# FintanH/rust-crdt

Hardware: AMD Instinct MI355X
Metric: replica-merges/sec (whole node) + achieved HBM GB/s as % of MI355X peak (higher is better)
Workload: dtype u64

## Files before the change

rust-crdt_amd/csrc/common.hpp:

```cpp
#pragma once

#include <hip/hip_runtime.h>

#include <cstdint>
#include <cstdio>
#include <algorithm>
#include <cstring>
#include <map>
#include <string>
#include <vector>

#include "crdt_gpu.h"
#include "shard_host.hpp"

namespace crdt {

using u64 = unsigned long long;
using u64x2 = unsigned long long __attribute__((ext_vector_type(2)));

constexpr int kWave = 64;

#ifndef CRDT_APPLY_WPE
#define CRDT_APPLY_WPE 0
#endif
#if CRDT_APPLY_WPE
#define CRDT_APPLY_ATTR __attribute__((amdgpu_waves_per_eu(CRDT_APPLY_WPE)))
#else
#define CRDT_APPLY_ATTR
#endif
constexpr int kBlock = 256;

struct KernelTimer {
  double total_ms = 0.0;
  uint64_t launches = 0;
};

struct Tune {
  int lub_blocks_per_cu = 1;
  int lub_grid = 0;
  int lub_persist_grid = 0;
  int lub_chunk_bytes = 512 << 10;
  int lub_min_steps = 16;
  int lub_interleave = 0;
  int lub_unroll = 8;
  int lub_nt = 1;
  int orswot_blocks_per_cu = 2;
  int orswot_unroll = 1;
  int orswot_mpt = 4;
  int merge_blocks_per_cu = 2;
  int merge_rows = 1;
  int map_glds = 1;
  int map_chunk = 16;
  int map_ring = 2;
  int map_spec = 1;
  int map_nt = 0;
  int map_scan2 = 0;
  int map_scan3 = 1;
  int map_rs = 1;
  int map_batch = 1;
  int map_sh = 0;
  int map_lazyv = 1;
  int map_st = 0;
  int shagree = 0;
  int map_diag = 0;
  int rows_blocks_per_cu = 0;
  int apply_hot_slots = 8;
  int map_apply_hot = 1 << 20;
  int map_forget_vec2 = 1;
  int map_pair_reg = 1;
  int pair_rows = 256;
  int pair_ur = 8;
  int pair_occ = 1;
  int map_forget_bpc = 1;
  int mvreg_forget_bpc = 32;
  int map_pair_pf = 0;
  int map_pair_nt = 1;
  int map_pair_bpc = 64;
  int merge_flat = 1;
  int merge_flat_u = 2;
  int merge_ppl = 8;
  int stage_kb = 262144;
  int wire_walk = 1;
  int wire_fill = 1;
  int host_stream = 1;
  int apply_lane = 1;
  int apply_fence = 0;
  int orswot_apply_pf = 0;
  int orswot_apply_stg = 0;
  int orswot_apply_l2pf = 0;
  int orswot_apply_meta = 1;
  int orswot_apply_hpf = 0;
  int map_counter_dma = 0;
  int map_counter_depth = 8;
  int map_counter_kpw = 0;
  int map_counter_cs = 1;
  int map_counter_cl = 0;
  int map_orswot_cs = 0;
  int map_orswot_wide = 0;
  int map_nested_lds = 1;
  int map_apply_meta = 1;
  int map_apply_pf = 1;
  int read_bpc = 0;
  int read_unroll = 8;
  int read_nt = 1;
  int eqv_ppl = 8;
  int eqv_bpc = 32;
};

struct PendingTiming {
  std::string name;
  hipEvent_t start, stop;
};

}

struct crdt_ctx {
  int device = 0;
  hipStream_t stream = nullptr;
  int cu_count = 256;
  bool timing = false;
  crdt::Tune tune;
  std::string last_error;
  void *scratch = nullptr;
  size_t scratch_bytes = 0;
  void *dscratch = nullptr;
  size_t dscratch_bytes = 0;
  unsigned *counters = nullptr;
  size_t counters_n = 0;
  void *pinned = nullptr;
  size_t pinned_bytes = 0;
  hipEvent_t pinned_done = nullptr;
  std::map<std::string, crdt::KernelTimer> timers;
  std::vector<crdt::PendingTiming> pending;
  std::vector<hipEvent_t> free_events;
  void *comm = nullptr;
  int nranks = 1, rank = 0;
  void (*comm_destroy)(void *) = nullptr;
  void *sbuf[8] = {};
  size_t sbuf_bytes[8] = {};
  bool has_ops = false;
  crdt_comm_ops ops{};
  hipStream_t astream = nullptr;
  hipEvent_t a_main = nullptr, a_done = nullptr;
  void *a_dev = nullptr, *a_host = nullptr;
  size_t a_rows = 0;
  std::string comm_note;
  void (*comm_release)(crdt_ctx *) = nullptr;
  crdt::shard_host::PlanCache plans;
  bool chk_pending = false;
  uint64_t chk_key = 0;
  void *chk_dev = nullptr;
  uint64_t *chk_host = nullptr;
  hipEvent_t chk_ev = nullptr;
  int (*comm_check)(crdt_ctx *) = nullptr;
  int mem_kind = CRDT_MEM_DEVICE;
  hipStream_t hstream = nullptr;
  void *hbuf[2] = {};
  size_t hbuf_bytes = 0;
  void *hacc = nullptr;
  size_t hacc_bytes = 0;
  hipEvent_t hcopied[2] = {}, hfree[2] = {};
};

namespace crdt {

int fail(crdt_ctx *ctx, int code, const char *fmt, ...);
int hip_fail(crdt_ctx *ctx, hipError_t e, const char *what);
int ensure_scratch(crdt_ctx *ctx, size_t bytes);
int ensure_dscratch(crdt_ctx *ctx, size_t bytes);
int ensure_counters(crdt_ctx *ctx, size_t n);
int stage_h2d(crdt_ctx *ctx, void *dst, const void *src, size_t bytes);
int device_fill(crdt_ctx *ctx, void *dst, size_t bytes, unsigned char byte);
void timing_begin(crdt_ctx *ctx, const char *name);
void timing_end(crdt_ctx *ctx);
void timing_add_host(crdt_ctx *ctx, const char *name, double ms);

struct DefPlan {
  const size_t *def_off;
  unsigned long long G, D, M, A, Mw;
  const u64 *def_clock, *def_members;
  const u64 *out_clock;
  u64 *out_entries;
  int apply_ceiling;
  u64 *hash;
  unsigned *surv;
  unsigned *nsurv;
  uint8_t *out_keep;
  u64 *out_members;
  u64 *tkey;
  unsigned *trep;
  unsigned long long tmask;
};
int launch_deferred(crdt_ctx *ctx, const size_t *host_def_off, DefPlan q, const u64 *dev_def_off = nullptr,
                    unsigned *status = nullptr);
int stage_def_off_dev(crdt_ctx *ctx, const u64 *src, size_t *dst, size_t G, size_t D, unsigned *status,
                      unsigned *flags);

enum class Op : int { Max = 0, Or = 1 };

template <Op OP>
__device__ __forceinline__ u64 join(u64 a, u64 b) {
// ... 103 lines not shown
```

rust-crdt_amd/csrc/ctx.cpp:

```cpp
#include <cstdarg>
#include <cstdlib>

#include "common.hpp"

namespace crdt {

static thread_local std::string g_orphan_error;

int fail(crdt_ctx *ctx, int code, const char *fmt, ...) {
  char buf[512];
  va_list ap;
  va_start(ap, fmt);
  vsnprintf(buf, sizeof buf, fmt, ap);
  va_end(ap);
  if (ctx) ctx->last_error = buf;
  else g_orphan_error = buf;
  return code;
}

int hip_fail(crdt_ctx *ctx, hipError_t e, const char *what) {
  return fail(ctx, CRDT_EHIP, "%s failed: %s (%d)", what, hipGetErrorString(e), (int)e);
}

int ensure_scratch(crdt_ctx *ctx, size_t bytes) {
// ... 30 lines not shown
  }
  ctx->dscratch_bytes = want;
  return CRDT_OK;
}

int ensure_counters(crdt_ctx *ctx, size_t n) {
  if (n <= ctx->counters_n) return CRDT_OK;
  if (ctx->counters) {
    (void)hipStreamSynchronize(ctx->stream);
    (void)hipFree(ctx->counters);
    ctx->counters = nullptr;
    ctx->counters_n = 0;
  }
  size_t want = n < 16384 ? 16384 : n * 2;
  hipError_t e = hipMalloc(&ctx->counters, want * sizeof(unsigned));
  if (e != hipSuccess) {
    ctx->counters = nullptr;
    return fail(ctx, CRDT_ENOMEM, "counter hipMalloc failed: %s", hipGetErrorString(e));
  }
  ctx->counters_n = want;
  return device_fill(ctx, ctx->counters, want * sizeof(unsigned), 0);
}

int stage_h2d(crdt_ctx *ctx, void *dst, const void *src, size_t bytes) {
  if (bytes == 0) return CRDT_OK;
  if (ctx->pinned_done) {
    hipError_t e = hipEventSynchronize(ctx->pinned_done);
    if (e != hipSuccess) return hip_fail(ctx, e, "hipEventSynchronize(pinned)");
  } else {
    hipError_t e = hipEventCreateWithFlags(&ctx->pinned_done, hipEventDisableTiming);
    if (e != hipSuccess) return hip_fail(ctx, e, "hipEventCreate(pinned)");
  }
  if (bytes > ctx->pinned_bytes) {
    if (ctx->pinned) (void)hipHostFree(ctx->pinned);
    ctx->pinned = nullptr;
    ctx->pinned_bytes = 0;
    size_t want = bytes < 65536 ? 65536 : bytes * 2;
    hipError_t e = hipHostMalloc(&ctx->pinned, want, hipHostMallocDefault);
    if (e != hipSuccess) return fail(ctx, CRDT_ENOMEM, "hipHostMalloc(%zu) failed", want);
    ctx->pinned_bytes = want;
  }
  std::memcpy(ctx->pinned, src, bytes);
  hipError_t e = hipMemcpyAsync(dst, ctx->pinned, bytes, hipMemcpyHostToDevice, ctx->stream);
  if (e != hipSuccess) return hip_fail(ctx, e, "hipMemcpyAsync(staged)");
  e = hipEventRecord(ctx->pinned_done, ctx->stream);
  if (e != hipSuccess) return hip_fail(ctx, e, "hipEventRecord(pinned)");
  return CRDT_OK;
}

__global__ void fill_u64_kernel(unsigned long long *p, size_t n, unsigned long long v) {
  for (size_t i = (size_t)blockIdx.x * blockDim.x + threadIdx.x; i < n; i += (size_t)gridDim.x * blockDim.x)
    p[i] = v;
}
__global__ void fill_u8_kernel(unsigned char *p, size_t n, unsigned char v) {
  for (size_t i = (size_t)blockIdx.x * blockDim.x + threadIdx.x; i < n; i += (size_t)gridDim.x * blockDim.x)
    p[i] = v;
}

int device_fill(crdt_ctx *ctx, void *dst, size_t bytes, unsigned char byte) {
  if (bytes == 0) return CRDT_OK;
  const bool wide = (reinterpret_cast<uintptr_t>(dst) % 8 == 0) && bytes % 8 == 0;
  const size_t n = wide ? bytes / 8 : bytes;
  size_t blocks = (n + kBlock - 1) / kBlock;
  const size_t cap = (size_t)ctx->cu_count * 8;
  if (blocks > cap) blocks = cap;
  if (wide)
    hipLaunchKernelGGL(fill_u64_kernel, dim3((unsigned)blocks), dim3(kBlock), 0, ctx->stream,
                       (unsigned long long *)dst, n, 0x0101010101010101ULL * byte);
  else
    hipLaunchKernelGGL(fill_u8_kernel, dim3((unsigned)blocks), dim3(kBlock), 0, ctx->stream,
                       (unsigned char *)dst, n, byte);
  hipError_t e = hipGetLastError();
  return e == hipSuccess ? CRDT_OK : hip_fail(ctx, e, "device_fill");
}

static hipEvent_t take_event(crdt_ctx *ctx) {
  if (!ctx->free_events.empty()) {
    hipEvent_t e = ctx->free_events.back();
    ctx->free_events.pop_back();
    return e;
  }
  hipEvent_t e = nullptr;
  (void)hipEventCreate(&e);
  return e;
}

void timing_begin(crdt_ctx *ctx, const char *name) {
  if (!ctx->timing) return;
  PendingTiming p;
  p.name = name;
  p.start = take_event(ctx);
  p.stop = take_event(ctx);
  (void)hipEventRecord(p.start, ctx->stream);
  ctx->pending.push_back(p);
}

void timing_end(crdt_ctx *ctx) {
  if (!ctx->timing || ctx->pending.empty()) return;
  (void)hipEventRecord(ctx->pending.back().stop, ctx->stream);
}

void timing_add_host(crdt_ctx *ctx, const char *name, double ms) {
  if (!ctx->timing) return;
  auto &t = ctx->timers[name];
  t.total_ms += ms;
  t.launches += 1;
}

static void drain_timings(crdt_ctx *ctx) {
  for (auto &p : ctx->pending) {
    (void)hipEventSynchronize(p.stop);
    float ms = 0.f;
    if (hipEventElapsedTime(&ms, p.start, p.stop) == hipSuccess) {
      auto &t = ctx->timers[p.name];
      t.total_ms += ms;
      t.launches += 1;
    }
    ctx->free_events.push_back(p.start);
    ctx->free_events.push_back(p.stop);
  }
  ctx->pending.clear();
}

}

using namespace crdt;

extern "C" {

static void apply_tune(crdt_ctx *ctx, const char *t) {
  std::string spec(t);
  size_t pos = 0;
  while (pos < spec.size()) {
    size_t end = spec.find(',', pos);
    if (end == std::string::npos) end = spec.size();
    std::string kv = spec.substr(pos, end - pos);
    size_t eq = kv.find('=');
    if (eq != std::string::npos) {
      std::string k = kv.substr(0, eq);
      int v = atoi(kv.c_str() + eq + 1);
      if (k == "bpc" && v > 0) ctx->tune.lub_blocks_per_cu = v;
      else if (k == "minsteps" && v > 0) ctx->tune.lub_min_steps = v;
      else if (k == "interleave") ctx->tune.lub_interleave = v != 0;
      else if (k == "unroll" && (v == 4 || v == 8 || v == 16 || v == 32)) ctx->tune.lub_unroll = v;
      else if (k == "nt") ctx->tune.lub_nt = v != 0;
      else if (k == "grid" && v > 0) ctx->tune.lub_grid = v;
      else if (k == "lubpg" && v >= 0) ctx->tune.lub_persist_grid = v;
      else if (k == "lubchunk" && v >= 0) ctx->tune.lub_chunk_bytes = v;
      else if (k == "mbpc" && v > 0) ctx->tune.merge_blocks_per_cu = v;
      else if (k == "mrows" && (v == 0 || v == 1)) ctx->tune.merge_rows = v;
      else if (k == "obpc" && v > 0) ctx->tune.orswot_blocks_per_cu = v;
      else if (k == "ounroll" && (v == 1 || v == 2 || v == 4)) ctx->tune.orswot_unroll = v;
      else if (k == "ompt" && (v == 4 || v == 8 || v == 16)) ctx->tune.orswot_mpt = v;
      else if (k == "mglds") ctx->tune.map_glds = v != 0;
      else if (k == "mchunk" && (v == 8 || v == 16)) ctx->tune.map_chunk = v;
      else if (k == "mring" && v >= 2 && v <= 4) ctx->tune.map_ring = v;
      else if (k == "mspec") ctx->tune.map_spec = v != 0;
      else if (k == "mnt") ctx->tune.map_nt = v != 0;
      else if (k == "mscan2") ctx->tune.map_scan2 = v != 0;
      else if (k == "mscan3") ctx->tune.map_scan3 = v != 0;
      else if (k == "mrs") ctx->tune.map_rs = v != 0;
      else if (k == "msh") ctx->tune.map_sh = v != 0;
      else if (k == "mst") ctx->tune.map_st = v != 0;
      else if (k == "shagree") ctx->tune.shagree = v != 0;
      else if (k == "mbatch") ctx->tune.map_batch = v != 0;
      else if (k == "mlazyv") ctx->tune.map_lazyv = v != 0;
      else if (k == "mdiag" && v >= 0) ctx->tune.map_diag = v;
      else if (k == "wwalk") ctx->tune.wire_walk = v != 0;
      else if (k == "hstream") ctx->tune.host_stream = v != 0;
      else if (k == "wfill") ctx->tune.wire_fill = v != 0;
      else if (k == "afence") ctx->tune.apply_fence = v != 0;
      else if (k == "alane") ctx->tune.apply_lane = v != 0;
      else if (k == "mfu" && (v == 1 || v == 2 || v == 4)) ctx->tune.merge_flat_u = v;
      else if (k == "mpnt") ctx->tune.map_pair_nt = v != 0;
      else if (k == "mppf") ctx->tune.map_pair_pf = v != 0;
      else if (k == "ohpf") ctx->tune.orswot_apply_hpf = v != 0;
      else if (k == "oal2") ctx->tune.orswot_apply_l2pf = v != 0;
      else if (k == "oameta") ctx->tune.orswot_apply_meta = v != 0;
      else if (k == "oastg") ctx->tune.orswot_apply_stg = v != 0;
      else if (k == "oapf") ctx->tune.orswot_apply_pf = v != 0;
      else if (k == "mcdep") ctx->tune.map_counter_depth = v >= 16 ? 16 : (v <= 4 ? 4 : 8);
      else if (k == "mckpw") ctx->tune.map_counter_kpw = v >= 4 ? 4 : (v >= 2 ? 2 : (v == 1 ? 1 : 0));
      else if (k == "mccs") ctx->tune.map_counter_cs = v ? 1 : 0;
      else if (k == "mccl") ctx->tune.map_counter_cl = v ? 1 : 0;
      else if (k == "mocs") ctx->tune.map_orswot_cs = v ? 1 : 0;
      else if (k == "mowide") ctx->tune.map_orswot_wide = v ? 1 : 0;
      else if (k == "nmlds") ctx->tune.map_nested_lds = v ? 1 : 0;
      else if (k == "mcdma") ctx->tune.map_counter_dma = v >= 16 ? 16 : (v > 0 ? 8 : 0);
      else if (k == "mapf") ctx->tune.map_apply_pf = v != 0;
      else if (k == "mameta") ctx->tune.map_apply_meta = v != 0;
      else if (k == "rbpc" && v > 0) ctx->tune.rows_blocks_per_cu = v;
      else if (k == "rdbpc" && v >= 0 && v <= 4096) ctx->tune.read_bpc = v;
      else if (k == "rdu" && (v == 4 || v == 8)) ctx->tune.read_unroll = v;
      else if (k == "rdnt") ctx->tune.read_nt = v != 0;
      else if (k == "hot" && v >= 0 && v <= 64) ctx->tune.apply_hot_slots = v;
      else if (k == "mhot" && v >= 0) ctx->tune.map_apply_hot = v;
      else if (k == "mfv2") ctx->tune.map_forget_vec2 = v != 0;
      else if (k == "stage_kb" && v >= 4) ctx->tune.stage_kb = v;
      else if (k == "mpreg" && v >= 0 && v <= 2) ctx->tune.map_pair_reg = v;
      else if (k == "prows" && (v == 64 || v == 128 || v == 256)) ctx->tune.pair_rows = v;
      else if (k == "pur" && (v == 2 || v == 4 || v == 8)) ctx->tune.pair_ur = v;
      else if (k == "pocc" && v >= 0 && v <= 8) ctx->tune.pair_occ = v;
      else if (k == "mppl" && v >= 1 && v <= 64) ctx->tune.merge_ppl = v;
      else if (k == "mflat" && v >= 0 && v <= 16) ctx->tune.merge_flat = v;
      else if (k == "mpbpc" && v >= 1 && v <= 4096) ctx->tune.map_pair_bpc = v;
      else if (k == "mfbpc" && v >= 1 && v <= 64) ctx->tune.map_forget_bpc = v;
      else if (k == "mvfbpc" && v >= 1 && v <= 64) ctx->tune.mvreg_forget_bpc = v;
      else if (k == "eqvppl" && v >= 1 && v <= 64) ctx->tune.eqv_ppl = v;
      else if (k == "eqvbpc" && v >= 1 && v <= 4096) ctx->tune.eqv_bpc = v;
    }
    pos = end + 1;
  }
}

int crdt_ctx_create(int device, crdt_ctx **out) {
  if (!out) return fail(nullptr, CRDT_EINVAL, "crdt_ctx_create: out is NULL");
  *out = nullptr;
  int n = 0;
  hipError_t e = hipGetDeviceCount(&n);
  if (e != hipSuccess || n == 0)
    return fail(nullptr, CRDT_EHIP, "crdt_ctx_create: no HIP device (%s)", hipGetErrorString(e));
  if (device < 0 || device >= n)
    return fail(nullptr, CRDT_EINVAL, "crdt_ctx_create: device %d out of range [0,%d)", device, n);
  e = hipSetDevice(device);
  if (e != hipSuccess) return hip_fail(nullptr, e, "hipSetDevice");
  auto *ctx = new crdt_ctx();
  ctx->device = device;
  hipDeviceProp_t prop;
  if (hipGetDeviceProperties(&prop, device) == hipSuccess && prop.multiProcessorCount > 0)
    ctx->cu_count = prop.multiProcessorCount;
  if (const char *t = getenv("CRDT_TUNE")) apply_tune(ctx, t);
  *out = ctx;
  return CRDT_OK;
}

int crdt_ctx_destroy(crdt_ctx *ctx) {
  if (!ctx) return CRDT_OK;
  (void)hipSetDevice(ctx->device);
  (void)hipStreamSynchronize(ctx->stream);
  for (auto &p : ctx->pending) {
    (void)hipEventDestroy(p.start);
    (void)hipEventDestroy(p.stop);
  }
  for (auto e : ctx->free_events) (void)hipEventDestroy(e);
  if (ctx->scratch) (void)hipFree(ctx->scratch);
  if (ctx->counters) (void)hipFree(ctx->counters);
  if (ctx->dscratch) (void)hipFree(ctx->dscratch);
  if (ctx->pinned) (void)hipHostFree(ctx->pinned);
  if (ctx->pinned_done) (void)hipEventDestroy(ctx->pinned_done);
  free_stage(ctx);
  if (ctx->comm && ctx->comm_destroy) ctx->comm_destroy(ctx->comm);
  if (ctx->comm_release) ctx->comm_release(ctx);
  for (void *b : ctx->sbuf)
    if (b) (void)hipFree(b);
  delete ctx;
  return CRDT_OK;
}

int crdt_ctx_set_stream(crdt_ctx *ctx, void *hip_stream) {
  CRDT_CHECK_CTX(ctx);
  ctx->stream = reinterpret_cast<hipStream_t>(hip_stream);
  return CRDT_OK;
}

int crdt_ctx_synchronize(crdt_ctx *ctx) {
  CRDT_CHECK_CTX(ctx);
  CRDT_HIP(ctx, hipSetDevice(ctx->device));
  CRDT_HIP(ctx, hipStreamSynchronize(ctx->stream));
  if (ctx->comm_check) return ctx->comm_check(ctx);
  return CRDT_OK;
}

const char *crdt_last_error(const crdt_ctx *ctx) {
  return ctx ? ctx->last_error.c_str() : g_orphan_error.c_str();
}

const char *crdt_version(void) { return "0.8.0"; }
int crdt_abi_version(void) { return CRDT_ABI_VERSION; }
const char *crdt_build_target(void) { return "gfx950"; }

int crdt_ctx_set_timing(crdt_ctx *ctx, int enable) {
  CRDT_CHECK_CTX(ctx);
  ctx->timing = enable != 0;
  return CRDT_OK;
}

int crdt_ctx_timing(crdt_ctx *ctx, const char *name, double *total_ms, uint64_t *launches) {
  CRDT_CHECK_CTX(ctx);
  if (!name) return fail(ctx, CRDT_EINVAL, "crdt_ctx_timing: name is NULL");
  drain_timings(ctx);
  auto it = ctx->timers.find(name);
  if (total_ms) *total_ms = it == ctx->timers.end() ? 0.0 : it->second.total_ms;
  if (launches) *launches = it == ctx->timers.end() ? 0 : it->second.launches;
  return CRDT_OK;
}

int crdt_ctx_timing_reset(crdt_ctx *ctx) {
  CRDT_CHECK_CTX(ctx);
  drain_timings(ctx);
  ctx->timers.clear();
  return CRDT_OK;
}

}

int crdt_ctx_tune(crdt_ctx *ctx, const char *spec) {
// ... 6 lines not shown
```

rust-crdt_amd/csrc/orswot.hip:

```cpp
#include "common.hpp"

namespace crdt {


template <int V>
struct OVec;
template <>
struct OVec<1> {
  using T = u64;
};
template <>
struct OVec<2> {
  using T = u64x2;
};

__device__ __forceinline__ u64 umax(u64 a, u64 b) { return a > b ? a : b; }

__device__ __forceinline__ u64 dot_join(u64 e1, u64 c1, u64 e2, u64 c2) {
  const u64 t0 = e1 == e2 ? e1 : 0;
  const u64 t1 = e1 > c2 ? e1 : 0;
  const u64 t2 = e2 > c1 ? e2 : 0;
  return umax(t0, umax(t1, t2));
}
__device__ __forceinline__ u64x2 dot_join(u64x2 e1, u64x2 c1, u64x2 e2, u64x2 c2) {
  u64x2 r;
  r.x = dot_join(e1.x, c1.x, e2.x, c2.x);
  r.y = dot_join(e1.y, c1.y, e2.y, c2.y);
  return r;
}
__device__ __forceinline__ u64x2 umax(u64x2 a, u64x2 b) {
  u64x2 r;
  r.x = umax(a.x, b.x);
  r.y = umax(a.y, b.y);
  return r;
}

struct OrPlan {
  const u64 *clock;
  const u64 *entries;
  long long c_rstride, c_gstride, e_mstride, e_rstride, e_gstride;
  unsigned long long G, R, M, A, Rs;
  int Wv, PW, MB, ncolblk, nmblk, S;
  u64 *part;
  unsigned *cnt;
  u64 *out_clock;
  u64 *out_entries;
  const u64 *init_clock;
  const u64 *init_entries;
  unsigned *viol;
};

#ifndef OR_VIOL_BALLOT
#define OR_VIOL_BALLOT 0
#endif
template <int V, int UR, int MPT>
__global__ __launch_bounds__(kBlock) void orswot_join_kernel(OrPlan p) {
  constexpr int kOrMPT = MPT;
  using VT = typename OVec<V>::T;
  __shared__ int s_flag;
  const int l = threadIdx.x;
  const unsigned b = blockIdx.x;
  const int s = b % p.S;
  unsigned u = b / p.S;
  const int cb = u % p.ncolblk;
  const unsigned rest = u / p.ncolblk;
  const int mb = rest % p.nmblk;
  const size_t g = rest / p.nmblk;
  const int cl = l % p.PW;
  const int ml = l / p.PW;
  const int col = cb * kBlock + cl;
  const bool active = ml < p.MB && col < p.Wv;
  const size_t mbase = (size_t)mb * p.MB * kOrMPT + ml;

  VT e[kOrMPT], c;
  bool mok[kOrMPT];
#pragma unroll
  for (int j = 0; j < kOrMPT; ++j) mok[j] = active && (mbase + (size_t)j * p.MB) < p.M;
  bool viol = false;
#if OR_VIOL_BALLOT
  u64 vmask = 0;
#endif
  auto gt = [](VT x, VT y) -> bool {
    if constexpr (V == 2) return (x.x > y.x) | (x.y > y.y);
    else return x > y;
  };
  auto start = [&](bool from_init) {
    c = VT(0);
#pragma unroll
    for (int j = 0; j < kOrMPT; ++j) e[j] = VT(0);
    if (!from_init || !p.init_clock || !active) return;
    c = reinterpret_cast<const VT *>(p.init_clock + g * p.A)[col];
    const VT *ie = reinterpret_cast<const VT *>(p.init_entries + g * p.M * p.A);
#pragma unroll
    for (int j = 0; j < kOrMPT; ++j)
      if (mok[j]) {
        e[j] = ie[(mbase + (size_t)j * p.MB) * (p.A / V) + col];
        viol |= gt(e[j], c);
      }
  };
  auto fold = [&](unsigned long long rbeg, unsigned long long rend) {
    const VT *cp = reinterpret_cast<const VT *>(p.clock + g * p.c_gstride + rbeg * p.c_rstride) + col;
    const VT *ep = reinterpret_cast<const VT *>(p.entries + g * p.e_gstride + rbeg * p.e_rstride +
                                                mbase * p.e_mstride) + col;
    const long long cstep = p.c_rstride / V;
    const long long estep = p.e_rstride / V;
    const long long mstep = (long long)p.MB * p.e_mstride / V;
    unsigned long long r = rbeg;
    for (; r + UR <= rend; r += UR) {
      VT c2[UR], e2[UR][kOrMPT];
#pragma unroll
      for (int q = 0; q < UR; ++q) {
        c2[q] = cp[q * cstep];
#pragma unroll
        for (int j = 0; j < kOrMPT; ++j)
          e2[q][j] = mok[j] ? __builtin_nontemporal_load(ep + q * estep + j * mstep) : VT(0);
      }
#pragma unroll
      for (int q = 0; q < UR; ++q) {
#pragma unroll
        for (int j = 0; j < kOrMPT; ++j) {
#if OR_VIOL_BALLOT
          if constexpr (V == 2) vmask |= __ballot(e2[q][j].x > c2[q].x) | __ballot(e2[q][j].y > c2[q].y);
          else vmask |= __ballot(e2[q][j] > c2[q]);
#else
          viol |= gt(e2[q][j], c2[q]);
#endif
          e[j] = dot_join(e[j], c, e2[q][j], c2[q]);
        }
        c = umax(c, c2[q]);
      }
      cp += UR * cstep;
      ep += UR * estep;
    }
    for (; r < rend; ++r) {
      const VT c2 = *cp;
      VT e2[kOrMPT];
#pragma unroll
      for (int j = 0; j < kOrMPT; ++j)
        e2[j] = mok[j] ? __builtin_nontemporal_load(ep + j * mstep) : VT(0);
#pragma unroll
      for (int j = 0; j < kOrMPT; ++j) {
        viol |= gt(e2[j], c2);
        e[j] = dot_join(e[j], c, e2[j], c2);
      }
      c = umax(c, c2);
      cp += cstep;
      ep += estep;
    }
  };

  start(s == 0);
  if (active) {
    const unsigned long long rbeg = (unsigned long long)s * p.Rs;
    fold(rbeg, min(p.R, rbeg + p.Rs));
  }
#if OR_VIOL_BALLOT
  viol |= vmask != 0;
#endif

  const size_t slab = (size_t)p.MB * kOrMPT * p.PW + p.PW;
  auto store_final = [&](void) {
    if (!active) return;
    VT *oe = reinterpret_cast<VT *>(p.out_entries + g * p.M * p.A);
#pragma unroll
    for (int j = 0; j < kOrMPT; ++j)
      if (mok[j]) oe[(mbase + (size_t)j * p.MB) * (p.A / V) + col] = e[j];
    if (mb == 0 && ml == 0) reinterpret_cast<VT *>(p.out_clock + g * p.A)[col] = c;
  };
  if (p.S == 1) {
    if (p.viol && __syncthreads_or(viol) && l == 0) atomicOr(p.viol + g, 1u);
    store_final();
    return;
  }
  VT *part = reinterpret_cast<VT *>(p.part) + ((size_t)u * p.S + s) * slab;
  if (active) {
#pragma unroll
    for (int j = 0; j < kOrMPT; ++j) part[(ml + j * p.MB) * p.PW + cl] = e[j];
    if (ml == 0) part[(size_t)p.MB * kOrMPT * p.PW + cl] = c;
  }
  asm volatile("s_waitcnt vmcnt(0)" ::: "memory");
  const int bviol = __syncthreads_or(viol);
  if (l == 0) {
    __builtin_amdgcn_fence(__ATOMIC_RELEASE, "agent");
    asm volatile("s_waitcnt vmcnt(0)" ::: "memory");
    const unsigned t = __hip_atomic_fetch_add(p.cnt + u, bviol ? 0x10001u : 1u, __ATOMIC_RELAXED,
                                              __HIP_MEMORY_SCOPE_AGENT);
    const int last = (t & 0xffffu) == (unsigned)p.S - 1;
    if (last) {
      __hip_atomic_store(p.cnt + u, 0u, __ATOMIC_RELAXED, __HIP_MEMORY_SCOPE_AGENT);
      __builtin_amdgcn_fence(__ATOMIC_ACQUIRE, "agent");
      asm volatile("s_waitcnt vmcnt(0)" ::: "memory");
      if ((bviol || (t >> 16)) && p.viol) atomicOr(p.viol + g, 1u);
    }
    s_flag = last | ((bviol || (t >> 16)) ? 2 : 0);
  }
  __syncthreads();
  if (!(s_flag & 1)) return;
  if (s_flag & 2) {
    start(true);
    if (active) fold(0, p.R);
#if OR_VIOL_BALLOT
    viol |= vmask != 0;
#endif
  } else if (active) {
    c = VT(0);
#pragma unroll
    for (int j = 0; j < kOrMPT; ++j) e[j] = VT(0);
    const VT *pp = reinterpret_cast<const VT *>(p.part) + (size_t)u * p.S * slab;
    for (int k = 0; k < p.S; ++k, pp += slab) {
      const VT c2 = pp[(size_t)p.MB * kOrMPT * p.PW + cl];
#pragma unroll
      for (int j = 0; j < kOrMPT; ++j) e[j] = dot_join(e[j], c, pp[(ml + j * p.MB) * p.PW + cl], c2);
      c = umax(c, c2);
    }
  }
  store_final();
}


__device__ __forceinline__ unsigned long long group_of(const size_t *off, unsigned long long G,
                                                       unsigned long long d) {
  unsigned long long lo = 0, hi = G;
  while (hi - lo > 1) {
    const unsigned long long mid = (lo + hi) / 2;
    if (off[mid] <= d) lo = mid;
    else hi = mid;
  }
  return lo;
}

__global__ __launch_bounds__(kBlock) void orswot_deferred_kernel(DefPlan p) {
  __shared__ u64 s_hash[kBlock / kWave];
  const unsigned long long d = blockIdx.x;
  const unsigned long long g = group_of(p.def_off, p.G, d);
  const u64 *rm = p.def_clock + d * p.A;
  const u64 *cf = p.out_clock + g * p.A;
  int greater = 0;
  u64 h = 0;
  for (unsigned long long a = threadIdx.x; a < p.A; a += kBlock) {
    const u64 x = rm[a];
    greater |= x > cf[a];
    u64 z = x * 0x9E3779B97F4A7C15ULL + a;
    z = (z ^ (z >> 30)) * 0xBF58476D1CE4E5B9ULL;
    z = (z ^ (z >> 27)) * 0x94D049BB133111EBULL;
    h += z ^ (z >> 31);
  }
  const int keep = __syncthreads_or(greater);
  for (int off = kWave / 2; off > 0; off >>= 1) h += __shfl_down(h, off, kWave);
  if ((threadIdx.x & (kWave - 1)) == 0) s_hash[threadIdx.x / kWave] = h;
  const u64 *bits = p.def_members + d * p.Mw;
  u64 *E = p.out_entries + g * p.M * p.A;
  for (unsigned long long w = 0; w < p.Mw && p.apply_ceiling; ++w) {
    u64 word = bits[w];
    while (word) {
      const int bit = __builtin_ctzll(word);
      word &= word - 1;
      const unsigned long long m = w * 64 + bit;
      if (m >= p.M) break;
      u64 *row = E + m * p.A;
      for (unsigned long long a = threadIdx.x; a < p.A; a += kBlock) {
        const u64 e = row[a];
        if (e != 0 && e <= rm[a]) row[a] = 0;
      }
    }
  }
  __syncthreads();
  if (threadIdx.x == 0) {
    u64 t = 0;
    for (int w = 0; w < kBlock / kWave; ++w) t += s_hash[w];
    p.hash[d] = t;
    if (keep) p.surv[atomicAdd(p.nsurv, 1u)] = (unsigned)d;
  }
}

__device__ __forceinline__ u64 dedup_key(u64 h, unsigned long long g) {
  u64 z = h ^ ((g + 1) * 0x9E3779B97F4A7C15ULL);
  z = (z ^ (z >> 31)) * 0xD6E8FEB86659FD93ULL;
  z ^= z >> 32;
  return z ? z : 1;
}

__device__ __forceinline__ unsigned long long dedup_slot(const DefPlan &p, u64 key, bool insert, unsigned d) {
  unsigned long long t = key & p.tmask;
  while (true) {
    const u64 cur = insert ? atomicCAS(p.tkey + t, 0ull, key) : p.tkey[t];
    if (cur == key || (insert && cur == 0)) return t;
    if (!insert && cur == 0) return ~0ull;
    t = (t + 1) & p.tmask;
  }
}

__global__ __launch_bounds__(kBlock) void orswot_dedup_insert_kernel(DefPlan p) {
  const unsigned k = blockIdx.x * blockDim.x + threadIdx.x;
  const unsigned n = *p.nsurv;
  if (k >= n) return;
  const unsigned d = p.surv[k];
  const u64 key = dedup_key(p.hash[d], group_of(p.def_off, p.G, d));
  atomicMin(p.trep + dedup_slot(p, key, true, d), d);
}

__global__ __launch_bounds__(kBlock) void orswot_dedup_kernel(DefPlan p) {
  const unsigned k = blockIdx.x * blockDim.x + threadIdx.x;
  const unsigned n = *p.nsurv;
  if (k >= n) return;
  const unsigned d = p.surv[k];
  const unsigned long long g = group_of(p.def_off, p.G, d);
  const u64 key = dedup_key(p.hash[d], g);
  const unsigned long long t = dedup_slot(p, key, false, d);
  const u64 *rm = p.def_clock + (size_t)d * p.A;
  auto same = [&](unsigned d2) {
    if (d2 < p.def_off[g] || d2 >= p.def_off[g + 1]) return false;
    const u64 *rm2 = p.def_clock + (size_t)d2 * p.A;
    for (unsigned long long a = 0; a < p.A; ++a)
      if (rm[a] != rm2[a]) return false;
    return true;
  };
  unsigned rep = t == ~0ull ? d : p.trep[t];
  if (rep != d && !same(rep)) {
    rep = d;
    for (unsigned j = 0; j < n; ++j) {
      const unsigned d2 = p.surv[j];
      if (d2 < rep && p.hash[d2] == p.hash[d] && same(d2)) rep = d2;
    }
  }
  if (rep == d) p.out_keep[d] = 1;
  const u64 *src = p.def_members + (size_t)d * p.Mw;
  u64 *dst = p.out_members + (size_t)rep * p.Mw;
  for (unsigned long long w = 0; w < p.Mw; ++w)
    if (src[w]) atomicOr(dst + w, src[w]);
}

static bool al16(const void *p) { return (reinterpret_cast<uintptr_t>(p) & 15) == 0; }

__global__ __launch_bounds__(kBlock) void def_off_check_kernel(const u64 *src, size_t *dst, unsigned long long G,
                                                               unsigned long long D, unsigned *status,
                                                               unsigned *flags) {
  const unsigned long long i = (unsigned long long)blockIdx.x * kBlock + threadIdx.x;
  if (i > G) return;
  const u64 v = src[i];
  bool bad = i == 0 ? v != 0 : (i == G ? v != D : v > D);
  if (i > 0 && src[i - 1] > v) bad = true;
  dst[i] = i == 0 ? 0 : (i == G ? D : (v > D ? D : v));
  if (bad) {
    if (status) atomicOr(status, 1u);
    if (flags) {
      if (i > 0) atomicOr(flags + i - 1, 2u);
      if (i < G) atomicOr(flags + i, 2u);
    }
  }
}

int stage_def_off_dev(crdt_ctx *ctx, const u64 *src, size_t *dst, size_t G, size_t D, unsigned *status,
                      unsigned *flags) {
  const size_t n = G + 1;
  hipLaunchKernelGGL(def_off_check_kernel, dim3((unsigned)((n + kBlock - 1) / kBlock)), dim3(kBlock), 0,
                     ctx->stream, src, dst, (unsigned long long)G, (unsigned long long)D, status, flags);
  CRDT_HIP(ctx, hipGetLastError());
  return CRDT_OK;
}

int launch_deferred(crdt_ctx *ctx, const size_t *host_def_off, DefPlan q, const u64 *dev_def_off, unsigned *status) {
  const size_t G = q.G, D = q.D;
  const size_t off_b = (G + 1) * sizeof(size_t);
  size_t T = 64;
  while (T < 2 * D) T <<= 1;
  const size_t off_pad = (off_b + 255) / 256 * 256;
  const size_t need = 256 + off_pad + D * 8 + D * 4 + 64 + T * 12;
  if (int rc = ensure_dscratch(ctx, need)) return rc;
  char *base = static_cast<char *>(ctx->dscratch);
  q.nsurv = reinterpret_cast<unsigned *>(base);
  q.def_off = reinterpret_cast<const size_t *>(base + 256);
  q.hash = reinterpret_cast<u64 *>(base + 256 + off_pad);
  q.surv = reinterpret_cast<unsigned *>(q.hash + D);
  q.tkey = reinterpret_cast<u64 *>(base + ((256 + off_pad + D * 12 + 63) / 64 * 64));
  q.trep = reinterpret_cast<unsigned *>(q.tkey + T);
  q.tmask = T - 1;
  if (int rc = device_fill(ctx, q.tkey, T * 8, 0)) return rc;
  if (int rc = device_fill(ctx, q.trep, T * 4, 0xFF)) return rc;
  if (int rc = device_fill(ctx, q.nsurv, 4, 0)) return rc;
  if (dev_def_off) {
    if (int rc = stage_def_off_dev(ctx, dev_def_off, (size_t *)q.def_off, G, D, status, nullptr)) return rc;
  } else {
    int rc = stage_h2d(ctx, (void *)q.def_off, host_def_off, off_b);
    if (rc) return rc;
  }
  if (int rc = device_fill(ctx, q.out_keep, D, 0)) return rc;
  if (int rc = device_fill(ctx, q.out_members, D * q.Mw * 8, 0)) return rc;
  hipLaunchKernelGGL(orswot_deferred_kernel, dim3((unsigned)D), dim3(kBlock), 0, ctx->stream, q);
  hipLaunchKernelGGL(orswot_dedup_insert_kernel, dim3((unsigned)((D + kBlock - 1) / kBlock)), dim3(kBlock), 0,
                     ctx->stream, q);
  hipLaunchKernelGGL(orswot_dedup_kernel, dim3((unsigned)((D + kBlock - 1) / kBlock)), dim3(kBlock), 0,
                     ctx->stream, q);
  CRDT_HIP(ctx, hipGetLastError());
  return CRDT_OK;
}

}

using namespace crdt;

static int orswot_lub_impl(crdt_ctx *ctx, const crdt_orswot_batch *in, const u64 *doff, size_t Ddev,
                           crdt_orswot_out *out, unsigned *status, const OrswotJoinExtra *ex = nullptr) {
  const size_t G = in->G, R = in->R, M = in->M, A = in->A;
  if (G == 0 || A == 0) return CRDT_OK;
  if (!out->clock || (M && !out->entries)) return fail(ctx, CRDT_EINVAL, "orswot_lub_many: NULL output");
  if (R > 0 && (!in->clock || (M && !in->entries)))
    return fail(ctx, CRDT_EINVAL, "orswot_lub_many: NULL input");
  if (in->entry_mstride < A && M > 1)
    return fail(ctx, CRDT_EINVAL, "orswot_lub_many: entry_mstride < A");
  if (A > (1u << 20) || M > (1ull << 32))
    return fail(ctx, CRDT_EUNSUPPORTED, "orswot_lub_many: A or M too large");
  CRDT_HIP(ctx, hipSetDevice(ctx->device));
  const size_t D = doff ? Ddev : (in->def_off && G > 0) ? in->def_off[G] - in->def_off[0] : 0;
  if (in->def_off && in->def_off[0] != 0)
    return fail(ctx, CRDT_EINVAL, "orswot_lub_many: def_off[0] must be 0");
  const size_t Mw = (M + 63) / 64;
  if (D > 0 && (!in->def_clock || !out->def_keep || (Mw && (!in->def_members || !out->def_members))))
    return fail(ctx, CRDT_EINVAL, "orswot_lub_many: deferred buffers missing");
  if (D > 0xffffffffULL) return fail(ctx, CRDT_EUNSUPPORTED, "orswot_lub_many: too many deferred");

  if (ex && ex->viol)
    if (int rc = device_fill(ctx, ex->viol, G * 4, 0)) return rc;
  if (R == 0 && ex && ex->init_clock) {
    CRDT_HIP(ctx, hipMemcpyAsync(out->clock, ex->init_clock, G * A * 8, hipMemcpyDeviceToDevice, ctx->stream));
    if (M)
      CRDT_HIP(ctx, hipMemcpyAsync(out->entries, ex->init_entries, G * M * A * 8, hipMemcpyDeviceToDevice,
                                   ctx->stream));
  } else if (R == 0) {
    int rc = device_fill(ctx, out->clock, G * A * 8, 0);
    if (!rc && M) rc = device_fill(ctx, out->entries, G * M * A * 8, 0);
    if (rc) return rc;
  } else if (M == 0) {
    if (int rc = lattice_lub_many(ctx, Op::Max, (const u64 *)in->clock, G, R, A, in->clock_rstride,
                                  in->clock_gstride, (u64 *)out->clock, A, 0))
      return rc;
  } else {
    const bool vec2 = A % 2 == 0 && in->clock_rstride % 2 == 0 && in->clock_gstride % 2 == 0 &&
                      in->entry_mstride % 2 == 0 && in->entry_rstride % 2 == 0 &&
                      in->entry_gstride % 2 == 0 && al16(in->clock) && al16(in->entries) &&
                      al16(out->clock) && al16(out->entries) &&
                      (!ex || !ex->init_clock || (al16(ex->init_clock) && al16(ex->init_entries)));
    const int V = vec2 ? 2 : 1;
    OrPlan p{};
    p.clock = (const u64 *)in->clock;
    p.entries = (const u64 *)in->entries;
    p.c_rstride = in->clock_rstride;
    p.c_gstride = in->clock_gstride;
    p.e_mstride = in->entry_mstride;
    p.e_rstride = in->entry_rstride;
    p.e_gstride = in->entry_gstride;
    p.G = G;
    p.R = R;
    p.M = M;
    p.A = A;
    p.Wv = (int)(A / V);
    p.PW = p.Wv <= kBlock ? p.Wv : kBlock;
    p.MB = kBlock / p.PW;
    p.ncolblk = (p.Wv + kBlock - 1) / kBlock;
    const int MPT = ctx->tune.orswot_mpt == 8 ? 8 : (ctx->tune.orswot_mpt == 16 ? 16 : 4);
    const size_t mpb = (size_t)p.MB * MPT;
    p.nmblk = (int)((M + mpb - 1) / mpb);
    p.out_clock = (u64 *)out->clock;
    p.out_entries = (u64 *)out->entries;
    if (ex) {
      p.init_clock = ex->init_clock;
      p.init_entries = ex->init_entries;
      p.viol = ex->viol;
    }
    const size_t units = G * (size_t)p.nmblk * p.ncolblk;
    const size_t target = (size_t)ctx->cu_count * ctx->tune.orswot_blocks_per_cu;
    size_t S = 1;
    if (units < target) {
      S = (target + units - 1) / units;
      size_t max_s = R / 8;
      if (max_s < 1) max_s = 1;
      if (S > max_s) S = max_s;
      if (S > 64) S = 64;
    }
    size_t Rs = (R + S - 1) / S;
    S = (R + Rs - 1) / Rs;
    p.S = (int)S;
    p.Rs = Rs;
    if (units * S > 0x7fffffffULL) return fail(ctx, CRDT_EUNSUPPORTED, "orswot_lub_many: grid too large");
    if (S > 1) {
      const size_t slab_b = (mpb * p.PW + p.PW) * V * 8;
      int rc = ensure_scratch(ctx, units * S * slab_b);
      if (rc) return rc;
      rc = ensure_counters(ctx, units);
      if (rc) return rc;
      p.cnt = ctx->counters;
      p.part = reinterpret_cast<u64 *>(ctx->scratch);
    }
    timing_begin(ctx, "orswot_join");
    const dim3 grid((unsigned)(units * S));
    const int UR = ctx->tune.orswot_unroll;
#define CRDT_ORJ(VV, UU, MM) hipLaunchKernelGGL((orswot_join_kernel<VV, UU, MM>), grid, dim3(kBlock), 0, ctx->stream, p)
    if (V == 2) {
      if (MPT == 4) {
        if (UR == 1) CRDT_ORJ(2, 1, 4);
        else if (UR == 4) CRDT_ORJ(2, 4, 4);
        else CRDT_ORJ(2, 2, 4);
      } else if (MPT == 8) {
        if (UR == 1) CRDT_ORJ(2, 1, 8);
        else CRDT_ORJ(2, 2, 8);
      } else {
        CRDT_ORJ(2, 1, 16);
      }
    } else {
      CRDT_ORJ(1, 2, 4);
    }
#undef CRDT_ORJ
    timing_end(ctx);
    CRDT_HIP(ctx, hipGetLastError());
  }

  if (D == 0) return CRDT_OK;
  DefPlan q{};
  q.G = G;
  q.D = D;
  q.M = M;
  q.A = A;
  q.Mw = Mw;
  q.def_clock = (const u64 *)in->def_clock;
  q.def_members = (const u64 *)in->def_members;
  q.out_clock = (const u64 *)out->clock;
  q.out_entries = (u64 *)out->entries;
  q.apply_ceiling = 1;
  q.out_keep = out->def_keep;
  q.out_members = (u64 *)out->def_members;
  return launch_deferred(ctx, in->def_off, q, doff, status);
}

namespace crdt {
int orswot_lub_many_ex(crdt_ctx *ctx, const crdt_orswot_batch *in, crdt_orswot_out *out, const OrswotJoinExtra &ex) {
  return orswot_lub_impl(ctx, in, nullptr, 0, out, nullptr, &ex);
}
}

extern "C" int crdt_orswot_lub_many(crdt_ctx *ctx, const crdt_orswot_batch *in,
                                    crdt_orswot_out *out) {
  if (ctx && ctx->mem_kind == CRDT_MEM_HOST) return crdt::orswot_lub_many_host(ctx, in, out);
  CRDT_CHECK_CTX(ctx);
  if (!in || !out) return fail(ctx, CRDT_EINVAL, "orswot_lub_many: NULL batch/out");
  return orswot_lub_impl(ctx, in, nullptr, 0, out, nullptr);
}

extern "C" int crdt_orswot_lub_many_doff(crdt_ctx *ctx, const crdt_orswot_batch *in, const uint64_t *def_off,
                                         size_t D, crdt_orswot_out *out, uint32_t *status) {
  CRDT_DEVICE_MEM_ONLY(ctx);
  CRDT_CHECK_CTX(ctx);
  if (!in || !out) return fail(ctx, CRDT_EINVAL, "orswot_lub_many_doff: NULL batch/out");
  if (in->def_off) return fail(ctx, CRDT_EINVAL, "orswot_lub_many_doff: in->def_off must be NULL");
  if (!def_off && D) return fail(ctx, CRDT_EINVAL, "orswot_lub_many_doff: D > 0 without def_off");
  CRDT_HIP(ctx, hipSetDevice(ctx->device));
  if (status)
    if (int rc = device_fill(ctx, status, sizeof(uint32_t), 0)) return rc;
  if (in->G == 0 || in->A == 0) return CRDT_OK;
  if (def_off && D == 0) {
    if (int rc = ensure_dscratch(ctx, (in->G + 1) * sizeof(size_t))) return rc;
    if (int rc = stage_def_off_dev(ctx, (const u64 *)def_off, (size_t *)ctx->dscratch, in->G, 0, status, nullptr))
      return rc;
    def_off = nullptr;
  }
  return orswot_lub_impl(ctx, in, (const u64 *)def_off, def_off ? D : 0, out, status);
}
```

Measured before the change: 2.290 billion.

## Software-pipeline ORSWOT join loads and specialize full tiles

Adds a register double-buffered fold in the ORSWOT join kernel: loads for the next PD replicas are issued before the current ones are joined, so memory latency overlaps compute. Full member tiles get a specialization without per-row bounds masks, and dot_join is simplified to two compares and one max. The default blocks-per-CU for the join drops from 2 to 1, and the V=1 path is forced to MPT=4. The prefetch buffers raise register pressure, and halving the grid may reduce latency hiding from occupancy.

```diff
diff --git a/rust-crdt_amd/csrc/common.hpp b/rust-crdt_amd/csrc/common.hpp
--- a/rust-crdt_amd/csrc/common.hpp
+++ b/rust-crdt_amd/csrc/common.hpp
@@ -44,9 +44,10 @@
   int lub_interleave = 0;
   int lub_unroll = 8;
   int lub_nt = 1;
-  int orswot_blocks_per_cu = 2;
+  int orswot_blocks_per_cu = 1;
   int orswot_unroll = 1;
   int orswot_mpt = 4;
+  int orswot_pipe = 2;
   int merge_blocks_per_cu = 2;
   int merge_rows = 1;
   int map_glds = 1;
diff --git a/rust-crdt_amd/csrc/ctx.cpp b/rust-crdt_amd/csrc/ctx.cpp
--- a/rust-crdt_amd/csrc/ctx.cpp
+++ b/rust-crdt_amd/csrc/ctx.cpp
@@ -206,6 +206,7 @@
       else if (k == "obpc" && v > 0) ctx->tune.orswot_blocks_per_cu = v;
       else if (k == "ounroll" && (v == 1 || v == 2 || v == 4)) ctx->tune.orswot_unroll = v;
       else if (k == "ompt" && (v == 4 || v == 8 || v == 16)) ctx->tune.orswot_mpt = v;
+      else if (k == "opipe" && v >= 0 && v <= 3) ctx->tune.orswot_pipe = v;
       else if (k == "mglds") ctx->tune.map_glds = v != 0;
       else if (k == "mchunk" && (v == 8 || v == 16)) ctx->tune.map_chunk = v;
       else if (k == "mring" && v >= 2 && v <= 4) ctx->tune.map_ring = v;
diff --git a/rust-crdt_amd/csrc/orswot.hip b/rust-crdt_amd/csrc/orswot.hip
--- a/rust-crdt_amd/csrc/orswot.hip
+++ b/rust-crdt_amd/csrc/orswot.hip
@@ -1,4 +1,7 @@
 #include "common.hpp"
+#include "orswot_join.hpp"
+
+#include <type_traits>
 
 namespace crdt {
 
@@ -16,16 +19,11 @@
 
 __device__ __forceinline__ u64 umax(u64 a, u64 b) { return a > b ? a : b; }
 
-__device__ __forceinline__ u64 dot_join(u64 e1, u64 c1, u64 e2, u64 c2) {
-  const u64 t0 = e1 == e2 ? e1 : 0;
-  const u64 t1 = e1 > c2 ? e1 : 0;
-  const u64 t2 = e2 > c1 ? e2 : 0;
-  return umax(t0, umax(t1, t2));
-}
+__device__ __forceinline__ u64 dot_join(u64 e1, u64 c1, u64 e2, u64 c2) { return dot_join2(e1, c1, e2, c2); }
 __device__ __forceinline__ u64x2 dot_join(u64x2 e1, u64x2 c1, u64x2 e2, u64x2 c2) {
   u64x2 r;
-  r.x = dot_join(e1.x, c1.x, e2.x, c2.x);
-  r.y = dot_join(e1.y, c1.y, e2.y, c2.y);
+  r.x = dot_join2(e1.x, c1.x, e2.x, c2.x);
+  r.y = dot_join2(e1.y, c1.y, e2.y, c2.y);
   return r;
 }
 __device__ __forceinline__ u64x2 umax(u64x2 a, u64x2 b) {
@@ -50,13 +48,12 @@
   unsigned *viol;
 };
 
-#ifndef OR_VIOL_BALLOT
-#define OR_VIOL_BALLOT 0
-#endif
-template <int V, int UR, int MPT>
+template <int V, int UR, int MPT, int PD>
 __global__ __launch_bounds__(kBlock) void orswot_join_kernel(OrPlan p) {
   constexpr int kOrMPT = MPT;
   using VT = typename OVec<V>::T;
+  using Full = std::integral_constant<bool, true>;
+  using Edge = std::integral_constant<bool, false>;
   __shared__ int s_flag;
   const int l = threadIdx.x;
   const unsigned b = blockIdx.x;
@@ -71,19 +68,27 @@
   const int col = cb * kBlock + cl;
   const bool active = ml < p.MB && col < p.Wv;
   const size_t mbase = (size_t)mb * p.MB * kOrMPT + ml;
+  const bool full = ((size_t)mb + 1) * p.MB * kOrMPT <= p.M;
 
   VT e[kOrMPT], c;
   bool mok[kOrMPT];
 #pragma unroll
   for (int j = 0; j < kOrMPT; ++j) mok[j] = active && (mbase + (size_t)j * p.MB) < p.M;
   bool viol = false;
-#if OR_VIOL_BALLOT
-  u64 vmask = 0;
-#endif
   auto gt = [](VT x, VT y) -> bool {
     if constexpr (V == 2) return (x.x > y.x) | (x.y > y.y);
     else return x > y;
   };
+  auto each_row = [&](auto &&fn) {
+    if (full) {
+#pragma unroll
+      for (int j = 0; j < kOrMPT; ++j) fn(j);
+    } else {
+#pragma unroll
+      for (int j = 0; j < kOrMPT; ++j)
+        if (mok[j]) fn(j);
+    }
+  };
   auto start = [&](bool from_init) {
     c = VT(0);
 #pragma unroll
@@ -91,80 +96,93 @@
     if (!from_init || !p.init_clock || !active) return;
     c = reinterpret_cast<const VT *>(p.init_clock + g * p.A)[col];
     const VT *ie = reinterpret_cast<const VT *>(p.init_entries + g * p.M * p.A);
-#pragma unroll
-    for (int j = 0; j < kOrMPT; ++j)
-      if (mok[j]) {
-        e[j] = ie[(mbase + (size_t)j * p.MB) * (p.A / V) + col];
-        viol |= gt(e[j], c);
-      }
+    each_row([&](int j) {
+      e[j] = ie[(mbase + (size_t)j * p.MB) * (p.A / V) + col];
+      viol |= gt(e[j], c);
+    });
   };
-  auto fold = [&](unsigned long long rbeg, unsigned long long rend) {
+  auto fold = [&](auto kind, unsigned long long rbeg, unsigned long long rend) {
+    constexpr bool kFull = decltype(kind)::value;
     const VT *cp = reinterpret_cast<const VT *>(p.clock + g * p.c_gstride + rbeg * p.c_rstride) + col;
     const VT *ep = reinterpret_cast<const VT *>(p.entries + g * p.e_gstride + rbeg * p.e_rstride +
                                                 mbase * p.e_mstride) + col;
     const long long cstep = p.c_rstride / V;
     const long long estep = p.e_rstride / V;
     const long long mstep = (long long)p.MB * p.e_mstride / V;
-    unsigned long long r = rbeg;
-    for (; r + UR <= rend; r += UR) {
-      VT c2[UR], e2[UR][kOrMPT];
-#pragma unroll
-      for (int q = 0; q < UR; ++q) {
-        c2[q] = cp[q * cstep];
-#pragma unroll
-        for (int j = 0; j < kOrMPT; ++j)
-          e2[q][j] = mok[j] ? __builtin_nontemporal_load(ep + q * estep + j * mstep) : VT(0);
+    auto load = [&](VT &c2, VT(&e2)[kOrMPT], int k) {
+      c2 = cp[k * cstep];
+#pragma unroll
+      for (int j = 0; j < kOrMPT; ++j) {
+        if constexpr (kFull) e2[j] = __builtin_nontemporal_load(ep + k * estep + j * mstep);
+        else e2[j] = mok[j] ? __builtin_nontemporal_load(ep + k * estep + j * mstep) : VT(0);
       }
-#pragma unroll
-      for (int q = 0; q < UR; ++q) {
-#pragma unroll
-        for (int j = 0; j < kOrMPT; ++j) {
-#if OR_VIOL_BALLOT
-          if constexpr (V == 2) vmask |= __ballot(e2[q][j].x > c2[q].x) | __ballot(e2[q][j].y > c2[q].y);
-          else vmask |= __ballot(e2[q][j] > c2[q]);
-#else
-          viol |= gt(e2[q][j], c2[q]);
-#endif
-          e[j] = dot_join(e[j], c, e2[q][j], c2[q]);
-        }
-        c = umax(c, c2[q]);
-      }
-      cp += UR * cstep;
-      ep += UR * estep;
-    }
-    for (; r < rend; ++r) {
-      const VT c2 = *cp;
-      VT e2[kOrMPT];
-#pragma unroll
-      for (int j = 0; j < kOrMPT; ++j)
-        e2[j] = mok[j] ? __builtin_nontemporal_load(ep + j * mstep) : VT(0);
+    };
+    auto join = [&](const VT &c2, const VT(&e2)[kOrMPT]) {
 #pragma unroll
       for (int j = 0; j < kOrMPT; ++j) {
         viol |= gt(e2[j], c2);
         e[j] = dot_join(e[j], c, e2[j], c2);
       }
       c = umax(c, c2);
-      cp += cstep;
-      ep += estep;
+    };
+    unsigned long long r = rbeg;
+    if constexpr (PD == 0) {
+      for (; r + UR <= rend; r += UR) {
+        VT c2[UR], e2[UR][kOrMPT];
+#pragma unroll
+        for (int q = 0; q < UR; ++q) load(c2[q], e2[q], q);
+#pragma unroll
+        for (int q = 0; q < UR; ++q) join(c2[q], e2[q]);
+        cp += UR * cstep;
+        ep += UR * estep;
+      }
+      if constexpr (UR > 1)
+        for (; r < rend; ++r) {
+          VT c2, e2[kOrMPT];
+          load(c2, e2, 0);
+          join(c2, e2);
+          cp += cstep;
+          ep += estep;
+        }
+    } else {
+      VT bc[PD], be[PD][kOrMPT];
+#pragma unroll
+      for (int q = 0; q < PD; ++q)
+        if (r + q < rend) load(bc[q], be[q], q);
+      for (; r + 2 * PD <= rend; r += PD) {
+#pragma unroll
+        for (int q = 0; q < PD; ++q) {
+          join(bc[q], be[q]);
+          load(bc[q], be[q], PD + q);
+        }
+        cp += PD * cstep;
+        ep += PD * estep;
+      }
+#pragma unroll
+      for (int q = 0; q < PD; ++q)
+        if (r + q < rend) {
+          join(bc[q], be[q]);
+          if (r + q + PD < rend) load(bc[q], be[q], PD + q);
+        }
+#pragma unroll
+      for (int q = 0; q < PD; ++q)
+        if (r + PD + q < rend) join(bc[q], be[q]);
     }
   };
 
   start(s == 0);
   if (active) {
     const unsigned long long rbeg = (unsigned long long)s * p.Rs;
-    fold(rbeg, min(p.R, rbeg + p.Rs));
-  }
-#if OR_VIOL_BALLOT
-  viol |= vmask != 0;
-#endif
+    const unsigned long long rend = min(p.R, rbeg + p.Rs);
+    if (full) fold(Full{}, rbeg, rend);
+    else fold(Edge{}, rbeg, rend);
+  }
 
   const size_t slab = (size_t)p.MB * kOrMPT * p.PW + p.PW;
   auto store_final = [&](void) {
     if (!active) return;
     VT *oe = reinterpret_cast<VT *>(p.out_entries + g * p.M * p.A);
-#pragma unroll
-    for (int j = 0; j < kOrMPT; ++j)
-      if (mok[j]) oe[(mbase + (size_t)j * p.MB) * (p.A / V) + col] = e[j];
+    each_row([&](int j) { oe[(mbase + (size_t)j * p.MB) * (p.A / V) + col] = e[j]; });
     if (mb == 0 && ml == 0) reinterpret_cast<VT *>(p.out_clock + g * p.A)[col] = c;
   };
   if (p.S == 1) {
@@ -198,10 +216,7 @@
   if (!(s_flag & 1)) return;
   if (s_flag & 2) {
     start(true);
-    if (active) fold(0, p.R);
-#if OR_VIOL_BALLOT
-    viol |= vmask != 0;
-#endif
+    if (active) fold(Edge{}, 0, p.R);
   } else if (active) {
     c = VT(0);
 #pragma unroll
@@ -215,6 +230,17 @@
     }
   }
   store_final();
+}
+
+template <int V, int UR, int MPT, int PD>
+static void orj_launch(crdt_ctx *ctx, dim3 grid, const OrPlan &p) {
+  hipLaunchKernelGGL((orswot_join_kernel<V, UR, MPT, PD>), grid, dim3(kBlock), 0, ctx->stream, p);
+}
+template <int V, int MPT>
+static void orj_launch_pipe(crdt_ctx *ctx, dim3 grid, const OrPlan &p, int PD) {
+  if (PD == 1) orj_launch<V, 1, MPT, 1>(ctx, grid, p);
+  else if (PD == 2) orj_launch<V, 1, MPT, 2>(ctx, grid, p);
+  else orj_launch<V, 1, MPT, 3>(ctx, grid, p);
 }
 
 
@@ -457,7 +483,7 @@
     p.PW = p.Wv <= kBlock ? p.Wv : kBlock;
     p.MB = kBlock / p.PW;
     p.ncolblk = (p.Wv + kBlock - 1) / kBlock;
-    const int MPT = ctx->tune.orswot_mpt == 8 ? 8 : (ctx->tune.orswot_mpt == 16 ? 16 : 4);
+    const int MPT = V == 1 ? 4 : ctx->tune.orswot_mpt == 8 ? 8 : (ctx->tune.orswot_mpt == 16 ? 16 : 4);
     const size_t mpb = (size_t)p.MB * MPT;
     p.nmblk = (int)((M + mpb - 1) / mpb);
     p.out_clock = (u64 *)out->clock;
@@ -494,22 +520,25 @@
     timing_begin(ctx, "orswot_join");
     const dim3 grid((unsigned)(units * S));
     const int UR = ctx->tune.orswot_unroll;
-#define CRDT_ORJ(VV, UU, MM) hipLaunchKernelGGL((orswot_join_kernel<VV, UU, MM>), grid, dim3(kBlock), 0, ctx->stream, p)
-    if (V == 2) {
+    const int PD = ctx->tune.orswot_pipe;
+    if (PD > 0 && UR == 1 && MPT != 16) {
+      if (V == 1) orj_launch_pipe<1, 4>(ctx, grid, p, PD);
+      else if (MPT == 4) orj_launch_pipe<2, 4>(ctx, grid, p, PD);
+      else orj_launch_pipe<2, 8>(ctx, grid, p, PD);
+    } else if (V == 2) {
       if (MPT == 4) {
-        if (UR == 1) CRDT_ORJ(2, 1, 4);
-        else if (UR == 4) CRDT_ORJ(2, 4, 4);
-        else CRDT_ORJ(2, 2, 4);
+        if (UR == 1) orj_launch<2, 1, 4, 0>(ctx, grid, p);
+        else if (UR == 4) orj_launch<2, 4, 4, 0>(ctx, grid, p);
+        else orj_launch<2, 2, 4, 0>(ctx, grid, p);
       } else if (MPT == 8) {
-        if (UR == 1) CRDT_ORJ(2, 1, 8);
-        else CRDT_ORJ(2, 2, 8);
+        if (UR == 1) orj_launch<2, 1, 8, 0>(ctx, grid, p);
+        else orj_launch<2, 2, 8, 0>(ctx, grid, p);
       } else {
-        CRDT_ORJ(2, 1, 16);
+        orj_launch<2, 1, 16, 0>(ctx, grid, p);
       }
     } else {
-      CRDT_ORJ(1, 2, 4);
-    }
-#undef CRDT_ORJ
+      orj_launch<1, 2, 4, 0>(ctx, grid, p);
+    }
     timing_end(ctx);
     CRDT_HIP(ctx, hipGetLastError());
   }
diff --git a/rust-crdt_amd/csrc/orswot_join.hpp b/rust-crdt_amd/csrc/orswot_join.hpp
--- /dev/null
+++ b/rust-crdt_amd/csrc/orswot_join.hpp
@@ -0,0 +1,27 @@
+#pragma once
+
+#if defined(__HIPCC__) || defined(__CUDACC__)
+#define CRDT_JOIN_HD __host__ __device__ inline
+#else
+#define CRDT_JOIN_HD inline
+#endif
+
+namespace crdt {
+
+using join_u64 = unsigned long long;
+
+CRDT_JOIN_HD join_u64 dot_join3(join_u64 e1, join_u64 c1, join_u64 e2, join_u64 c2) {
+  const join_u64 t0 = e1 == e2 ? e1 : 0;
+  const join_u64 t1 = e1 > c2 ? e1 : 0;
+  const join_u64 t2 = e2 > c1 ? e2 : 0;
+  const join_u64 t01 = t0 > t1 ? t0 : t1;
+  return t01 > t2 ? t01 : t2;
+}
+
+CRDT_JOIN_HD join_u64 dot_join2(join_u64 e1, join_u64 c1, join_u64 e2, join_u64 c2) {
+  const join_u64 a = ((e1 > c2) | (e1 == e2)) ? e1 : 0;
+  const join_u64 b = e2 > c1 ? e2 : 0;
+  return a > b ? a : b;
+}
+
+}
```

Measured after the change: 2.283 billion. No clear change (-0.3%).
